# PacificBiosciences/portello

Hardware: AMD Instinct MI355X
Metric: lifted HiFi reads/sec (whole node) (higher is better)
Workload: dtype int32; 1 GPU; wgs30x; reads_total=2000000, reads_this_rank=2000000, read_len_mean=15000, items_per_gpu=2065417, in_ops_per_gpu=62827345, out_ops_per_gpu=56590310, large_items_per_gpu=0, mid_items_per_gpu=0, retry_items_per_gpu=0, lane_items_per_gpu=2065417, heavy_lane_items_per_gpu=0, seq_fmt=bam4, parallelism=one read set, 20 Mb windows dealt to 1 ranks by input ops, gather=none, launched_by=single process

## Files before the change

### portello_amd/csrc/engine.hip

```cpp
#include <hip/hip_runtime.h>

#include <plo_wave.hpp>
#include <stdio.h>
#include <string.h>

#include <algorithm>
#include <chrono>
#include <map>
#include <mutex>
#include <string>
#include <vector>

#include "enumerate.hpp"
#include "finish_core.hpp"
#include "records_core.hpp"
#include "index_pack.hpp"
#include "inflate.hpp"
#include "deflate.hpp"
#include "lift_core.hpp"
#include "lane_core.hpp"
#include "lane_stream.hpp"

using namespace plo;

// ... 96 lines not shown
        bad |= (uint32_t)__shfl_xor((int)bad, (int)d, 64);
    }
    if (!live || sub != 0) return;
    if (bad) n = 0;
    seg_reflen[s] = (int)part;
    seg_readlen[s] = rpart > 0xfffffffeull ? 0xffffffffu : (uint32_t)rpart;
    seg_nm[s] = (c1 - c0) - pairs;
    seg_cnt[s] = n;
}

__global__ void k_item_emit(DevIndex ix, DevBatch bt, DevWork wk, uint32_t stages, const uint32_t *seg_off, int *seg_reflen, uint32_t item_cap, uint32_t *err) {
    uint32_t s = blockIdx.x * blockDim.x + threadIdx.x;
    if (s >= bt.n_segs) return;
    const uint32_t o0 = seg_off[s], o1 = seg_off[s + 1];
    if (o1 > item_cap) {
        if (o1 > o0) atomicOr(err, (uint32_t)VERR_CAP);
        return;
    }
    const int ref_len = seg_reflen[s];
    SegInfo si;
    seg_info_level0(si, bt, wk, stages, s);
    if (o0 == o1) return;
    seg_info_level1(si, ix, bt, wk, stages, s);
    emit_segment_items(ix, wk, stages, s, o0, (long long)ref_len, si);
}

__global__ __launch_bounds__(64) void k_map_build(const uint32_t *seg_cigar, const uint32_t *seg_cigar_off, const int64_t *seg_pos, uint32_t n_segments,
                                                  const uint32_t *kv_off, KV *kv, int *counts) {
    for (uint32_t g = blockIdx.x; g < n_segments; g += gridDim.x) {
        const uint32_t c0 = seg_cigar_off[g], c1 = seg_cigar_off[g + 1];
        const int cnt = build_segment_map_wave(seg_cigar + c0, c1 - c0, (long long)seg_pos[g], kv ? kv + kv_off[g] : nullptr);
        if (counts && threadIdx.x == 0) counts[g] = cnt;
    }
}

__global__ void k_item_desc(DevIndex ix, DevBatch bt, DevWork wk, uint32_t stages, const uint32_t *in_seg, const uint32_t *in_cseg,
                            uint32_t *err) {
    uint32_t i = blockIdx.x * blockDim.x + threadIdx.x;
    if (i >= wk.n_items) return;
    uint32_t seg = in_seg[i];
    {
        bool ok = seg < bt.n_segs;
        if (ok) {
            uint32_t contig = bt.seg_contig[seg];
            ok = contig < ix.n_contigs && in_cseg[i] < ix.contig_seg_off[contig + 1] - ix.contig_seg_off[contig];
        }
        if (!ok) {
            atomicOr(err, (uint32_t)VERR_INDEX);
            wk.item_cls[i] = 2u;
            wk.item_nin[i] = 0u;
            return;
        }
    }
    build_item_desc(ix, bt, wk, stages, i, seg, in_cseg[i], segment_ref_len(bt, seg));
}

constexpr int SCAN_THREADS = 256;
constexpr int SCAN_PER_THREAD = 8;
constexpr int SCAN_BLOCK = SCAN_THREADS * SCAN_PER_THREAD;

__device__ __forceinline__ unsigned block_scan_incl(unsigned v, unsigned *wave_tot , unsigned &block_total) {
    int lane = threadIdx.x & 63, w = threadIdx.x >> 6;
    unsigned inc = (unsigned)wv::scan_add((int)v);
    if (lane == 63) wave_tot[w] = inc;
    __syncthreads();
    unsigned base = 0;
// ... 1160 lines not shown
        d_chrom_ref, d_chrom_ref_len, d_read_len;
    DevBuf o_status, o_flip, o_mapq, o_chrom, o_pos, o_coff, o_clen, o_cigar, o_dense_off, o_cigar_dense, wave_stats;
    DevBuf fast_blk;
    bool fast_timing = false;
    bool scan_chain = false;
    bool fast_fuse = true;
    bool phase_events = true;
    bool fast_no_events = false;
    DevBuf i_read_rev, i_read_len, i_read_off, i_seq, i_seg_read, i_seg_contig, i_seg_pos, i_seg_fwd, i_seg_coff, i_cigar,
        i_item_seg, i_item_cseg;
    HostBuf h_item_seg, h_item_cseg, h_status, h_flip, h_mapq, h_chrom, h_pos, h_coff, h_clen, h_cigar, h_counters, h_miss, h_side;
    hipEvent_t ev[7] = {nullptr, nullptr, nullptr, nullptr, nullptr, nullptr, nullptr};
    hipStream_t copy_stream = nullptr;
    hipEvent_t ev_seq = nullptr;
    hipEvent_t ev_cls = nullptr;
    bool seq_pending = false;
    bool ev_big = false, ev_mid = false;
    uint64_t dense_total = 0;
    plo_timing timing{};
    unsigned long long phase_cycles[12] = {0};
    int window = 256, big_thresh = 176, cap = 320;
    bool adaptive = true;
    int n_cus = 256;
    int tile_waves = TILE_WAVES;
    bool small_window_tight = false;
    int lane_max_w = 192;
    int lane_capw = 3072;
    bool lane_sort = true;
    DevBuf lane_ticket;
    uint32_t lane_epoch = 0;
    int lane_static_rounds = 0;
    int lane_tail_rounds = 1;
    int lane_kvs = LANE_KVS;
    bool lane_h16 = false;
    bool lane_stats = false;
    int lane_sort_window = LANE_SORT_WINDOW;
    bool lane_budget = false;
    int lane_budget_window = 512;
    bool lane_stream = true;
    bool fast = true;
    uint32_t fast_ns_cap = 0, fast_item_cap = 0, fast_n0 = 0, fast_n1 = 0;
    uint32_t fast_ref_items = 0, fast_ref_ns = 0;
    bool fast_launch_bound = true;
    uint32_t item_cap_now = 0;
    uint32_t fast_extra_syncs = 0;
    bool fast_light_only = false;
    uint32_t lane_groups_cap = 0;
    int lane_heavy_min = -1;
    int lane_heavy_ratio = 50000;
    int lane_stream_ratio = 30000;
    int mid_waves = 16;
    int mid_cap_max = 4096;
};

#define HIP_TRY(ctx, call)                                                                      \
    do {                                                                                        \
        hipError_t _e = (call);                                                                 \
        if (_e != hipSuccess) {                                                                 \
            (ctx)->err = std::string(#call) + ": " + hipGetErrorString(_e);                     \
            return (_e == hipErrorOutOfMemory) ? PLO_ERR_OUT_OF_MEMORY : PLO_ERR_HIP;           \
        }                                                                                       \
    } while (0)

static thread_local std::string g_index_err;

template <class T>
// ... 57 lines not shown
        if (upload(tmp, cg, &d_cg) != hipSuccess || upload(tmp, cgoff, &d_cgoff) != hipSuccess || upload(tmp, spos, &d_pos) != hipSuccess ||
            upload(tmp, cnt, &d_cnt) != hipSuccess) {
            drop_tmp();
            return fail(PLO_ERR_HIP);
        }
        if (ns) hipLaunchKernelGGL(k_map_build, dim3(std::min<uint32_t>(ns, 65535u * 16u)), dim3(64), 0, 0, d_cg, d_cgoff, d_pos, ns, (const uint32_t *)nullptr,
                                   (KV *)nullptr, (int *)d_cnt);
        if (hipMemcpy(cnt.data(), d_cnt, cnt.size() * 4, hipMemcpyDeviceToHost) != hipSuccess) {
            drop_tmp();
            return fail(PLO_ERR_HIP);
        }
        ix->host.cs_kv_off.assign(ns + 1, 0);
        for (uint32_t g = 0; g < ns; ++g) {
            if (cnt[g] < 0) {
                g_index_err = "contig segment coordinate outside the 31-bit BAM range or invalid CIGAR op code";
                drop_tmp();
                return fail(PLO_ERR_RANGE);
            }
            ix->host.cs_kv_off[g + 1] = ix->host.cs_kv_off[g] + (uint32_t)cnt[g];
        }
        if (upload(ix->owned, h.cs_kv_off, &d.cs_kv_off) != hipSuccess) {
            drop_tmp();
            return fail(PLO_ERR_HIP);
        }
        void *kvp = nullptr;
        if (hipMalloc(&kvp, std::max<size_t>((size_t)h.cs_kv_off[ns] * sizeof(KV), 16)) != hipSuccess) {
            drop_tmp();
            return fail(PLO_ERR_OUT_OF_MEMORY);
        }
        ix->owned.push_back(kvp);
        d.kv = (const KV *)kvp;
        if (ns) hipLaunchKernelGGL(k_map_build, dim3(std::min<uint32_t>(ns, 65535u * 16u)), dim3(64), 0, 0, d_cg, d_cgoff, d_pos, ns, d.cs_kv_off, (KV *)kvp,
                                   (int *)nullptr);
        hipError_t e = hipDeviceSynchronize();
        drop_tmp();
        if (e != hipSuccess) return fail(PLO_ERR_HIP);
    }
    if (upload(ix->owned, h.cs_chrom, &d.cs_chrom) != hipSuccess) return fail(PLO_ERR_HIP);
    if (upload(ix->owned, h.cs_is_fwd, &d.cs_is_fwd) != hipSuccess) return fail(PLO_ERR_HIP);
    if (upload(ix->owned, h.cs_mapq, &d.cs_mapq) != hipSuccess) return fail(PLO_ERR_HIP);
    if (upload(ix->owned, h.cs_start, &d.cs_start) != hipSuccess) return fail(PLO_ERR_HIP);
    if (upload(ix->owned, h.cs_end, &d.cs_end) != hipSuccess) return fail(PLO_ERR_HIP);
    if (upload(ix->owned, h.contig_seg_off, &d.contig_seg_off) != hipSuccess) return fail(PLO_ERR_HIP);
    if (upload(ix->owned, h.contig_len, &d.contig_len) != hipSuccess) return fail(PLO_ERR_HIP);
    if (upload(ix->owned, h.chrom_len, &d.chrom_len) != hipSuccess) return fail(PLO_ERR_HIP);
    d.n_contigs = desc->n_contigs;
    d.n_segments = desc->n_segments;
    d.n_chroms = desc->n_chroms;
    std::vector<const uint8_t *> chrom_ptr(desc->n_chroms, nullptr), rev_ptr(desc->n_contigs, nullptr);
    for (uint32_t c = 0; c < desc->n_chroms; ++c) {
        const uint8_t *src = desc->chrom_seq[c];
        if (!src && desc->chrom_len[c] > 0) return fail(PLO_ERR_INVALID_ARG);
        if (desc->seq_mem == PLO_MEM_DEVICE) {
            chrom_ptr[c] = src;
        } else {
            void *p = nullptr;
            size_t bytes = std::max<size_t>((size_t)desc->chrom_len[c], 16);
            if (hipMalloc(&p, bytes) != hipSuccess) return fail(PLO_ERR_OUT_OF_MEMORY);
            ix->owned.push_back(p);
            if (desc->chrom_len[c] > 0 && hipMemcpy(p, src, (size_t)desc->chrom_len[c], hipMemcpyHostToDevice) != hipSuccess)
                return fail(PLO_ERR_HIP);
            chrom_ptr[c] = (const uint8_t *)p;
        }
    }
    for (uint32_t c = 0; c < desc->n_contigs; ++c) {
        const uint8_t *src = desc->rev_contig_seq ? desc->rev_contig_seq[c] : nullptr;
// ... 73 lines not shown
    (void)hipFuncSetAttribute((const void *)k_lift_tiles, hipFuncAttributeMaxDynamicSharedMemorySize, 160 * 1024);
    (void)hipFuncSetAttribute((const void *)k_lift_tiles_sp, hipFuncAttributeMaxDynamicSharedMemorySize, 160 * 1024);
    (void)hipFuncSetAttribute((const void *)k_lift_tiles_c256, hipFuncAttributeMaxDynamicSharedMemorySize, 160 * 1024);
    (void)hipFuncSetAttribute((const void *)k_lift_retry_sp, hipFuncAttributeMaxDynamicSharedMemorySize, 160 * 1024);
    (void)hipFuncSetAttribute((const void *)k_lift_mid_sp<8>, hipFuncAttributeMaxDynamicSharedMemorySize, 160 * 1024);
    (void)hipFuncSetAttribute((const void *)k_lift_mid_sp<16>, hipFuncAttributeMaxDynamicSharedMemorySize, 160 * 1024);
    if (getenv("PLO_DEBUG")) {
        for (int cap : {256, 320, 384, 512}) {
            int nb = -1;
            size_t lds = ((tile_mem_bytes(cap) + 15) & ~(size_t)15) * TILE_WAVES;
            hipError_t e = hipOccupancyMaxActiveBlocksPerMultiprocessor(&nb, (const void *)k_lift_tiles, TILE_WAVES * 64, lds);
            fprintf(stderr, "[plo] cap %d: dynamic LDS %zu B/block -> %d blocks/CU (%s)\n", cap, lds, nb, hipGetErrorString(e));
        }
    }
    (void)hipFuncSetAttribute((const void *)k_lift_mid<8>, hipFuncAttributeMaxDynamicSharedMemorySize, 160 * 1024);
    (void)hipFuncSetAttribute((const void *)k_lift_mid<16>, hipFuncAttributeMaxDynamicSharedMemorySize, 160 * 1024);
    if (const char *e = getenv("PLO_MID_WAVES")) {
        int v = atoi(e);
        c->mid_waves = v >= 16 ? 16 : (v >= 8 ? 8 : 0);
    }
    if (const char *e = getenv("PLO_MID_CAP")) c->mid_cap_max = std::min(4096, std::max(256, atoi(e) & ~63));
    (void)hipFuncSetAttribute((const void *)k_lift_retry, hipFuncAttributeMaxDynamicSharedMemorySize, 160 * 1024);
    (void)hipFuncSetAttribute((const void *)k_lift_lanes, hipFuncAttributeMaxDynamicSharedMemorySize, 160 * 1024);
    (void)hipFuncSetAttribute((const void *)k_lift_lanes_sp, hipFuncAttributeMaxDynamicSharedMemorySize, 160 * 1024);
    (void)hipFuncSetAttribute((const void *)k_lift_lanes_stats, hipFuncAttributeMaxDynamicSharedMemorySize, 160 * 1024);
    (void)hipFuncSetAttribute((const void *)k_lift_lanes16, hipFuncAttributeMaxDynamicSharedMemorySize, 160 * 1024);
    (void)hipFuncSetAttribute((const void *)k_lift_lanes16_stats, hipFuncAttributeMaxDynamicSharedMemorySize, 160 * 1024);
    if (const char *e = getenv("PLO_LANE_MAX_W")) c->lane_max_w = atoi(e);
    if (const char *e = getenv("PLO_LANE_SORT")) c->lane_sort = atoi(e) != 0;
    if (const char *e = getenv("PLO_LANE_STATIC")) c->lane_static_rounds = atoi(e);
    if (const char *e = getenv("PLO_LANE_STATS")) c->lane_stats = atoi(e) != 0;
    if (const char *e = getenv("PLO_LANE_H16")) c->lane_h16 = atoi(e) != 0;
    if (const char *e = getenv("PLO_LANE_TAIL")) c->lane_tail_rounds = std::max(0, atoi(e));
    if (const char *e = getenv("PLO_LANE_KVS")) c->lane_kvs = std::min(LANE_KVS_MAX, std::max(64, atoi(e) & ~63));
    if (!c->lane_h16) c->lane_kvs = std::min(c->lane_kvs, LANE_KVS);
    if (const char *e = getenv("PLO_LANE_SORT_WINDOW")) c->lane_sort_window = c->lane_budget_window = std::min(2048, std::max(64, atoi(e) & ~63));
    if (const char *e = getenv("PLO_LANE_BUDGET")) c->lane_budget = atoi(e) != 0;
    if (const char *e = getenv("PLO_LANE_HEAVY_MIN")) c->lane_heavy_min = atoi(e);
    if (const char *e = getenv("PLO_LANE_HEAVY_RATIO")) c->lane_heavy_ratio = std::max(0, atoi(e));
    if (const char *e = getenv("PLO_LANE_STREAM_RATIO")) c->lane_stream_ratio = std::max(1, atoi(e));
    if (const char *e = getenv("PLO_FAST_PATH")) c->fast = atoi(e) != 0;
    if (const char *e = getenv("PLO_SCAN_CHAIN")) c->scan_chain = atoi(e) != 0;
    if (const char *e = getenv("PLO_FAST_LAUNCH_BOUND")) c->fast_launch_bound = atoi(e) != 0;
    if (const char *e = getenv("PLO_FAST_FUSE")) c->fast_fuse = atoi(e) != 0;
    if (const char *e = getenv("PLO_RECORDS_BYTECOPY")) c->rec_bytecopy = atoi(e) != 0;
    if (const char *e = getenv("PLO_PHASE_EVENTS")) c->phase_events = atoi(e) != 0;
    if (const char *e = getenv("PLO_LANE_CAPW")) c->lane_capw = std::min(40000, std::max(64, atoi(e))) & ~3;
    if (c->lane_max_w + LANE_SLACK > c->lane_capw) c->lane_max_w = c->lane_capw - LANE_SLACK;
    if (const char *e = getenv("PLO_TILE_WAVES")) c->tile_waves = std::min(TILE_WAVES, std::max(1, atoi(e)));
    if (const char *e = getenv("PLO_WINDOW")) c->window = std::max(16, atoi(e)), c->adaptive = false;
    if (const char *e = getenv("PLO_BIG_THRESH")) c->big_thresh = std::max(1, atoi(e)), c->adaptive = false;
    if (const char *e = getenv("PLO_CAP")) c->cap = std::max(64, atoi(e)), c->adaptive = false;
    *out = c;
    return PLO_OK;
}

void plo_ctx_destroy(plo_ctx *c) {
    if (!c) return;
    (void)hipSetDevice(c->ix->device);
    (void)hipStreamSynchronize(c->stream);
    DevBuf *bufs[] = {&c->f_flag, &c->f_bin, &c->f_end, &c->f_prim, &c->f_isoff, &c->f_iqoff, &c->f_iread, &c->f_nl, &c->f_pitem,
                      &c->f_uflag, &c->f_rsoff, &c->f_rqoff, &c->f_su, &c->f_qu, &c->f_soff, &c->f_qoff, &c->f_rseq, &c->f_rqual, &c->f_fflag, &c->f_frank, &c->f_flist, &c->sa_len, &c->sa_off, &c->sa_text, &c->r_plan, &c->r_size, &c->r_start, &c->r_partial, &c->r_recoff, &c->r_out, &c->r_err, &c->z_slots, &c->z_size, &c->z_off, &c->z_partial, &c->z_tok, &c->z_out, &c->z_err,
                      &c->item_region, &c->lane_groups, &c->lane_ticket, &c->misc, &c->whist, &c->cls_partial, &c->lane_scratch, &c->item_cls, &c->retry_list, &c->perm, &c->nin_p, &c->seg_reflen, &c->seg_readlen, &c->seg_nm, &c->seg_cnt, &c->seg_off, &c->scan_partial, &c->item_seg, &c->item_cseg, &c->item_nin, &c->op_prefix,
                      &c->counters, &c->big_list, &c->huge_list, &c->verr, &c->scratch, &c->tile_lo, &c->d_n_m, &c->d_in_off, &c->d_n_in, &c->d_pos1,
                      &c->d_w0, &c->d_w1, &c->d_kv0, &c->d_kv1, &c->d_flags, &c->d_contig, &c->d_seq_len, &c->d_seq_off, &c->d_shift_ref,
                      &c->d_shift_ref_len, &c->d_chrom_ref, &c->d_chrom_ref_len, &c->d_read_len, &c->o_status, &c->o_flip, &c->o_mapq, &c->o_chrom, &c->o_pos,
// ... 400 lines not shown
            for (; b > 0; --b) {
                if (above + hist[b] > allow) break;
                above += hist[b];
            }
            int thresh = std::min(std::max(176, (b + 1) * WHIST_STEP), (WHIST_BINS - 1) * WHIST_STEP);
            c->big_thresh = thresh;
            c->cap = thresh <= 176 && !sp && !getenv("PLO_NO_SMALL_CAP") ? TILE_CAP_SMALL : (thresh <= 256 ? 320 : (thresh + 144 + 63) & ~63);
            c->window = c->cap - (c->cap == TILE_CAP_SMALL && !c->small_window_tight ? 32 : 64);
            c->tile_waves = c->cap <= 320 ? TILE_WAVES : (c->cap <= 448 ? 2 : 1);
            if (getenv("PLO_DEBUG_GEOMETRY"))
                fprintf(stderr, "[plo] batch geometry: thresh %d cap %d window %d tile_waves %d (max weight %u, %llu items beyond the 0.2 %% cut)\n", thresh, c->cap,
                        c->window, c->tile_waves, max_nin, above);
        }
    }
    const uint32_t n_tiles = total_ops / (uint32_t)c->window + 1;
    if (n_items > n_small && !heavy_lanes) {
        HIP_TRY(c, c->tile_lo.ensure((size_t)(n_tiles + 1) * 4));
        hipLaunchKernelGGL(k_tile_bounds, dim3((n_tiles + 1 + 255) / 256), dim3(256), 0, st, (const uint32_t *)c->op_prefix.as<uint32_t>(),
                           n_items, n_tiles, c->window, n_small, c->tile_lo.as<uint32_t>());
    }
    wk.tile_lo = c->tile_lo.as<uint32_t>();
    wk.n_small = n_small;
    HIP_TRY(c, hipEventRecord(c->ev[1], st));

    uint32_t lane_gs = 64, lane_nblk = 0;
    const size_t lane_lds = (size_t)(c->lane_capw + 2 * c->lane_kvs) * 4 * LANE_WAVES;
    if (n_small) {
        int occ = 1;
        if (hipOccupancyMaxActiveBlocksPerMultiprocessor(&occ, sp ? (const void *)k_lift_lanes_sp : (const void *)k_lift_lanes, LANE_WAVES * 64, lane_lds) != hipSuccess || occ < 1)
            occ = 1;
        const uint32_t n0 = h_cls[0], n1 = h_cls[1];
        const uint32_t slots = (uint32_t)(c->n_cus * occ) * LANE_WAVES;
        while (lane_gs > 8u && (n0 + lane_gs / 2 - 1) / (lane_gs / 2) + (n1 + lane_gs / 2 - 1) / (lane_gs / 2) <= slots) lane_gs >>= 1;
        if (const char *e = getenv("PLO_LANE_GROUP")) lane_gs = std::min(64u, std::max(1u, (uint32_t)atoi(e)));
        const uint32_t groups = (n0 + lane_gs - 1) / lane_gs + (n1 + lane_gs - 1) / lane_gs;
        lane_nblk = std::min<uint32_t>((groups + LANE_WAVES - 1) / LANE_WAVES, (uint32_t)(c->n_cus * occ));
        lane_nblk = (lane_nblk + 7u) & ~7u;
    }
    size_t want_cigar = (size_t)all_ops * 2 + (size_t)n_items * 8 + 4096 + (size_t)std::min<uint32_t>(n_tiles + 1024, (uint32_t)c->n_cus * 16) * SLAB_OPS +
                        (size_t)lane_nblk * LANE_WAVES * SLAB_OPS;
    if (c->o_cigar.cap < want_cigar * 4) HIP_TRY(c, c->o_cigar.ensure(want_cigar * 4));

    if (c->seq_pending) {
        HIP_TRY(c, hipStreamWaitEvent(st, c->ev_seq, 0));
        c->seq_pending = false;
    }
    unsigned long long *hc = c->h_counters.as<unsigned long long>();
    uint32_t n_big = 0, n_retry = 0, n_mid = 0, n_huge = 0, n_miss = 0, heavy_kernel = 0;
    float miss_ms = 0.f;
    for (int attempt = 0;; ++attempt) {
        wk.out_cigar = c->o_cigar.as<uint32_t>();
        wk.out_cap = c->o_cigar.cap / 4;
        HIP_TRY(c, hipMemsetAsync(c->counters.p, 0, CNT_N * 8, st));
        if (attempt == 0) HIP_TRY(c, hipEventRecord(c->ev[1], st));
        wk.slab_pre = 0;
        wk.slab_offset = 0;
        if (n_small) {
            const uint32_t n0 = h_cls[0], n1 = h_cls[1];
            const bool budget = c->lane_sort && wk.item_region && lane_gs == 64u;
            uint32_t lane_groups_cap_now = 0;
            if (attempt == 0 && c->lane_sort) {
                const uint32_t ch = (uint32_t)(budget ? c->lane_budget_window : c->lane_sort_window);
                const uint32_t chunks = (n0 + ch - 1) / ch + (n1 + ch - 1) / ch;
                uint32_t *n_groups_dev = c->misc.as<uint32_t>() + 32;
                if (budget) {
                    const uint32_t per_group = std::min<uint32_t>(64u, std::max<uint32_t>(1u, (uint32_t)c->lane_capw / (uint32_t)std::max(1, c->lane_max_w)));
                    const size_t max_groups = (size_t)chunks * (ch / per_group + 2);
// ... 322 lines not shown
    HIP_TRY(c, c->h_counters.ensure(FB_BYTES));
    uint8_t *const fb = c->fast_blk.as<uint8_t>();
    uint32_t *const misc_d = (uint32_t *)fb, *const verr_d = (uint32_t *)(fb + FB_VERR);
    unsigned long long *const counters_d = (unsigned long long *)(fb + FB_COUNTERS);
    const bool ev_on = c->phase_events;
    if (ev_on) HIP_TRY(c, hipEventRecord(c->ev[0], st));
    HIP_TRY(c, hipMemsetAsync(fb, 0, fb_bytes, st));
    hipLaunchKernelGGL(k_seg_count, dim3((unsigned)(((unsigned long long)ns * SEG_LANES + 255) / 256)), dim3(256), 0, st, ix, bt, c->seg_cnt.as<uint32_t>(),
                       c->seg_reflen.as<int>(), c->seg_readlen.as<uint32_t>(), c->seg_nm.as<uint32_t>(), verr_d);
    if (chain) {
        hipLaunchKernelGGL(k_scan_chain, dim3(scan_nb), dim3(SCAN_THREADS), 0, st, (const uint32_t *)c->seg_cnt.as<uint32_t>(), ns, c->seg_off.as<uint32_t>(),
                           (unsigned long long *)(fb + FB_BYTES), (uint32_t *)(fb + FB_TICKET));
    } else {
        plo_status s = scan_u32(c, c->seg_cnt.as<uint32_t>(), ns, c->seg_off.as<uint32_t>());
        if (s != PLO_OK) return s;
    }
    const uint32_t *n_dev = c->seg_off.as<uint32_t>() + ns, *totals_dev = misc_d;
    DevWork wk;
    fill_work(c, wk, cap);
    wk.counters = counters_d;
    hipLaunchKernelGGL(k_item_emit, dim3((ns + 255) / 256), dim3(256), 0, st, ix, bt, wk, stages, (const uint32_t *)c->seg_off.as<uint32_t>(), c->seg_reflen.as<int>(),
                       cap, verr_d);
    const uint32_t cls_nb = (cap + CLS_BLOCK - 1) / CLS_BLOCK;
    HIP_TRY(c, c->cls_partial.ensure((size_t)std::max(1u, cls_nb) * 6 * 4));
    hipLaunchKernelGGL(k_cls_hist, dim3(cls_nb), dim3(CLS_THREADS), 0, st, (const uint32_t *)c->item_cls.as<uint32_t>(), (const uint32_t *)c->item_nin.as<uint32_t>(), cap,
                       cls_nb, c->cls_partial.as<uint32_t>(), n_dev);
    hipLaunchKernelGGL(k_permute2_s, dim3(cls_nb), dim3(CLS_THREADS), 0, st, (const uint32_t *)c->item_cls.as<uint32_t>(), (const uint32_t *)c->item_nin.as<uint32_t>(),
                       (const uint32_t *)c->cls_partial.as<uint32_t>(), misc_d, cap, cls_nb, c->perm.as<uint32_t>(), c->nin_p.as<uint32_t>(),
                       c->adaptive ? (uint32_t)((WHIST_BINS - 1) * WHIST_STEP) : 0xffffffffu, n_dev);
    if (ev_on) HIP_TRY(c, hipEventRecord(c->ev[1], st));
    uint32_t lane_gs = 64, lane_nblk = 0;
    const size_t lane_lds = (size_t)(c->lane_capw + 2 * c->lane_kvs) * 4 * LANE_WAVES;
    {
        int occ = 1;
        if (hipOccupancyMaxActiveBlocksPerMultiprocessor(&occ, (const void *)k_lift_lanes, LANE_WAVES * 64, lane_lds) != hipSuccess || occ < 1) occ = 1;
        const uint32_t n0 = c->fast_n0, n1 = c->fast_n1, slots = (uint32_t)(c->n_cus * occ) * LANE_WAVES;
        while (lane_gs > 8u && (n0 + lane_gs / 2 - 1) / (lane_gs / 2) + (n1 + lane_gs / 2 - 1) / (lane_gs / 2) <= slots) lane_gs >>= 1;
        if (const char *e = getenv("PLO_LANE_GROUP")) lane_gs = std::min(64u, std::max(1u, (uint32_t)atoi(e)));
        const uint32_t groups = cap / lane_gs + 2;
        lane_nblk = std::min<uint32_t>((groups + LANE_WAVES - 1) / LANE_WAVES, (uint32_t)(c->n_cus * occ));
        lane_nblk = (lane_nblk + 7u) & ~7u;
    }
    const uint32_t ch = (uint32_t)c->lane_sort_window;
    hipLaunchKernelGGL(k_chunk_sort_w, dim3((cap / ch + 2u + 3u) / 4u), dim3(256), 0, st, c->perm.as<uint32_t>(), (const uint32_t *)c->d_n_m.as<uint32_t>(),
                       (const uint32_t *)c->d_w0.as<uint32_t>(), (const uint32_t *)c->d_w1.as<uint32_t>(), 0u, 0u, ch, totals_dev);
    wk.out_cigar = c->o_cigar.as<uint32_t>();
    wk.out_cap = c->o_cigar.cap / 4;
    wk.slab_pre = 1u;
    wk.slab_offset = (unsigned long long)lane_nblk * LANE_WAVES * SLAB_OPS;
    wk.n_small = cap;
    wk.lane_n_groups = misc_d + 32;
    wk.stat_base = 0;
    uint32_t stat_used = lane_nblk * LANE_WAVES;
    if (wk.slab_offset + SLAB_OPS > wk.out_cap) {
        fallback = true;
        return PLO_OK;
    }
    if (c->seq_pending) {
        HIP_TRY(c, hipStreamWaitEvent(st, c->ev_seq, 0));
        c->seq_pending = false;
    }
    lane_ticket_arm(c, wk, (c->fast_n0 + lane_gs - 1) / lane_gs + (c->fast_n1 + lane_gs - 1) / lane_gs, lane_nblk * LANE_WAVES);
    hipLaunchKernelGGL(lane_kernel_of(c, stages, false), dim3(lane_nblk), dim3(LANE_WAVES * 64), lane_lds, st, ix, bt, wk, stages, 0u, 0u, lane_gs, c->lane_capw, totals_dev);
    HIP_TRY(c, hipGetLastError());
    if (ev_on) HIP_TRY(c, hipEventRecord(c->ev[4], st));
    {
        const int retry_cap = 320;
        const uint32_t lds = (uint32_t)((tile_mem_bytes(retry_cap) + 15) & ~(size_t)15), nw = (uint32_t)c->n_cus * 2u;
#ifdef PLO_PHASE_TIMING
        const bool fuse = false;
#else
// ... 847 lines not shown
```

### portello_amd/csrc/enumerate.hpp

```cpp
#pragma once
#include <plo_wave.hpp>

#include "lift_types.hpp"

namespace plo {

#ifdef PLO_EMULATOR
alignas(16) static const uint32_t plo_safe_words[8] = {0, 0, 0, 0, 0, 0, 0, 0};
#else
alignas(16) static __device__ const uint32_t plo_safe_words[8] = {0, 0, 0, 0, 0, 0, 0, 0};
#endif

#ifdef PLO_EMULATOR
#define PLO_LEVEL_END(...)
#else
#define PLO_LV_(x) "v"(x)
#define PLO_LV1(a) PLO_LV_(a)
#define PLO_LV2(a, ...) PLO_LV_(a), PLO_LV1(__VA_ARGS__)
#define PLO_LV3(a, ...) PLO_LV_(a), PLO_LV2(__VA_ARGS__)
#define PLO_LV4(a, ...) PLO_LV_(a), PLO_LV3(__VA_ARGS__)
#define PLO_LV5(a, ...) PLO_LV_(a), PLO_LV4(__VA_ARGS__)
#define PLO_LV6(a, ...) PLO_LV_(a), PLO_LV5(__VA_ARGS__)
#define PLO_LV7(a, ...) PLO_LV_(a), PLO_LV6(__VA_ARGS__)
#define PLO_LV8(a, ...) PLO_LV_(a), PLO_LV7(__VA_ARGS__)
#define PLO_LV9(a, ...) PLO_LV_(a), PLO_LV8(__VA_ARGS__)
#define PLO_LV_N(_1, _2, _3, _4, _5, _6, _7, _8, _9, n, ...) PLO_LV##n
#define PLO_LEVEL_END(...) asm volatile("" ::PLO_LV_N(__VA_ARGS__, 9, 8, 7, 6, 5, 4, 3, 2, 1)(__VA_ARGS__))
#endif

PLO_DEV long long segment_ref_len(const DevBatch &bt, uint32_t seg) {
    uint32_t c0 = bt.seg_cigar_off[seg], c1 = bt.seg_cigar_off[seg + 1];
    long long r = 0;
    for (uint32_t i = c0; i < c1; ++i) {
        uint32_t c = bt.cigar[i];
        if ((0x18D >> (c & 15u)) & 1) r += (long long)(c >> 4);
    }
    return r;
}

PLO_DEV uint32_t segment_read_len_sat(const DevBatch &bt, uint32_t seg) {
    uint32_t c0 = bt.seg_cigar_off[seg], c1 = bt.seg_cigar_off[seg + 1];
    unsigned long long r = 0;
    for (uint32_t i = c0; i < c1; ++i) {
        uint32_t c = bt.cigar[i];
        if ((0x1B3 >> (c & 15u)) & 1) r += (unsigned long long)(c >> 4);
    }
    return r > 0xfffffffeull ? 0xffffffffu : (uint32_t)r;
}

PLO_DEV uint32_t segment_n_merged(const DevBatch &bt, uint32_t seg) {
    uint32_t c0 = bt.seg_cigar_off[seg], c1 = bt.seg_cigar_off[seg + 1];
    uint32_t n = 0;
    bool prev = false;
    for (uint32_t i = c0; i < c1; ++i) {
        const bool m = ((0x181u >> (bt.cigar[i] & 15u)) & 1u) != 0u;
        n += (m && prev) ? 0u : 1u;
        prev = m;
    }
    return n;
}
// ... 40 lines not shown
        int mid = (int)(((unsigned)lo + (unsigned)hi) >> 1);
        if (kv[mid].key < x)
            lo = mid + 1;
        else
            hi = mid;
    }
    return lo;
}

PLO_DEV int kv_lower_bound_near(const KV *kv, int lo, int hi, int x) {
    {
        int k[8];
#pragma unroll
        for (int j = 0; j < 8; ++j) k[j] = (lo + j < hi ? kv + (lo + j) : (const KV *)plo_safe_words)->key;
        int c = 0;
#pragma unroll
        for (int j = 0; j < 8; ++j) c += ((lo + j < hi) & (k[j] < x)) ? 1 : 0;
        if (c < 8 || lo + 8 >= hi) return lo + c;
        lo += 8;
    }
    int step = 1;
    while (lo < hi) {
        int probe = lo + step - 1;
        if (probe >= hi) break;
        if (kv[probe].key < x) {
            lo = probe + 1;
            step <<= 1;
        } else {
            hi = probe;
            break;
        }
    }
    return kv_lower_bound(kv, lo, hi, x);
}

PLO_HD int build_segment_map(const uint32_t *cigar, uint32_t n, long long ref_pos, KV *out) {
    long long read_pos = 0, match_len = 0;
    int cnt = 0;
    int last_key = -1;
    bool bad = false;
    for (uint32_t i = 0; i <= n; ++i) {
        uint32_t c = i < n ? cigar[i] : 4u;
        int t = (int)(c & 15u);
        long long len = (long long)(c >> 4);
        if (t > 8) bad = true;
        bool is_m = (t == OP_M || t == OP_EQ || t == OP_X);
        if (is_m) {
            match_len += len;
        } else if (match_len > 0) {
            if (read_pos > 0x7ffffff0LL || ref_pos > 0x7ffffff0LL || ref_pos - match_len < 0) {
                bad = true;
            } else {
                int k0 = (int)(read_pos - match_len), v0 = (int)(ref_pos - match_len), k1 = (int)read_pos;
                if (cnt > 0 && last_key == k0) {
                    if (out) out[cnt - 1].val = v0;
                } else {
                    if (out) {
                        out[cnt].key = k0;
                        out[cnt].val = v0;
                    }
                    ++cnt;
                }
                if (out) {
                    out[cnt].key = k1;
                    out[cnt].val = NONE32;
                }
// ... 90 lines not shown
    uint64_t seq_off, revseq;
    bool seg_fwd, read_rev;
};
PLO_DEV void seg_info_level0(SegInfo &s, const DevBatch &bt, const DevWork &wk, uint32_t stages, uint32_t seg) {
    s.contig = bt.seg_contig[seg];
    s.read = bt.seg_read[seg];
    s.in_off = bt.seg_cigar_off[seg];
    s.n_in = bt.seg_cigar_off[seg + 1];
    s.pos = (long long)bt.seg_pos[seg];
    s.n_m = wk.seg_nm ? wk.seg_nm[seg] : 0u;
    s.read_len = wk.seg_readlen ? wk.seg_readlen[seg] : 0u;
    const uint32_t sf = (stages & PLO_STAGE_STRAND) ? (uint32_t)bt.seg_is_fwd[seg] : 0u;
    PLO_LEVEL_END(s.contig, s.read, s.in_off, s.n_in, s.pos, s.n_m, s.read_len, sf);
    s.seg_fwd = sf != 0u;
    s.n_in -= s.in_off;
}
PLO_DEV void seg_info_level1(SegInfo &s, const DevIndex &ix, const DevBatch &bt, const DevWork &wk, uint32_t stages, uint32_t seg) {
    s.g0 = ix.contig_seg_off[s.contig];
    s.g1 = ix.contig_seg_off[s.contig + 1];
    s.contig_len = ix.contig_len[s.contig];
    s.revseq = ix.contig_revseq ? (uint64_t)(uintptr_t)ix.contig_revseq[s.contig] : 0ull;
    s.seq_len = bt.read_seq_len[s.read];
    s.seq_off = bt.read_seq_off[s.read];
    const uint32_t rr = (stages & PLO_STAGE_STRAND) ? (uint32_t)bt.read_is_reverse[s.read] : 0u;
    PLO_LEVEL_END(s.g0, s.g1, s.contig_len, s.revseq, s.seq_len, s.seq_off, rr);
    s.read_rev = rr != 0u;
    if (!wk.seg_nm) s.n_m = segment_n_merged(bt, seg);
    if (!wk.seg_readlen) s.read_len = segment_read_len_sat(bt, seg);
}
struct CsegInfo {
    int start, end;
    uint32_t kv0, kv1, chrom;
    uint8_t is_fwd, mapq;
};
PLO_DEV CsegInfo cseg_info(const DevIndex &ix, uint32_t gseg) {
    CsegInfo c;
    c.start = ix.cs_start[gseg];
    c.end = ix.cs_end[gseg];
    c.kv0 = ix.cs_kv_off[gseg];
    c.kv1 = ix.cs_kv_off[gseg + 1];
    c.chrom = ix.cs_chrom[gseg];
    const uint32_t f = ix.cs_is_fwd[gseg], q = ix.cs_mapq[gseg];
    PLO_LEVEL_END(c.start, c.end, c.kv0, c.kv1, c.chrom, f, q);
    c.is_fwd = (uint8_t)f;
    c.mapq = (uint8_t)q;
    return c;
}

PLO_DEV void build_item_desc(const DevIndex &ix, const DevWork &wk, uint32_t stages, uint32_t i, uint32_t seg, uint32_t cseg, long long ref_len,
                             const SegInfo &s, const CsegInfo &c) {
    const bool contig_fwd = c.is_fwd != 0;
    bool flip = false, rev = false;
    if (stages & PLO_STAGE_STRAND) {
        const bool changes = s.read_rev == s.seg_fwd;
        flip = (!contig_fwd) != changes;
        rev = !contig_fwd;
    }
    const long long pos1 = rev ? (long long)s.contig_len - (s.pos + ref_len) : s.pos;
    const int kv0 = (int)c.kv0, kv1 = (int)c.kv1;
    const long long lo = pos1 < -0x7fffffffLL ? -0x7fffffffLL : pos1;
    const long long hi = pos1 + ref_len > 0x7fffffffLL ? 0x7fffffffLL : pos1 + ref_len;
    int slo = kv0, shi = kv1;
    kv_upper_bound_narrow(ix.kv, slo, shi, (int)lo);
    const uint64_t chrom_ref = (uint64_t)(uintptr_t)ix.chrom_seq[c.chrom];
    const int chrom_ref_len = ix.chrom_len[c.chrom];
    const int ub = kv_upper_bound_tail(ix.kv, slo, shi, (int)lo);
    PLO_LEVEL_END(chrom_ref, chrom_ref_len, ub);
    const int w0 = ub - 1 > kv0 ? ub - 1 : kv0;
    const int w1 = kv_lower_bound_near(ix.kv, w0, kv1, (int)hi);
    const bool do_shift = (stages & PLO_STAGE_LSHIFT) && (!(stages & PLO_STAGE_STRAND) || !contig_fwd);
    const bool merges = do_shift || (stages & PLO_STAGE_LIFTOVER);
    const int region = lane_region_dwords((int)(merges ? s.n_m : s.n_in), w0, w1);
    wk.item_seg[i] = seg;
    wk.item_cseg[i] = cseg;
    wk.item_nin[i] = (uint32_t)item_weight((int)s.n_in, w0, w1, kv1);
    wk.item_cls[i] = (do_shift ? 1u : 0u) | ((wk.lane_max_w < 0 || region > wk.lane_max_w) ? 2u : 0u);
    if (wk.item_region) wk.item_region[i] = (uint32_t)region;
    wk.d.n_m[i] = s.n_m;
    wk.d.in_off[i] = s.in_off;
    wk.d.n_in[i] = s.n_in;
    wk.d.pos1[i] = (int)pos1;
    wk.d.w0[i] = (uint32_t)w0;
    wk.d.w1[i] = (uint32_t)w1;
    wk.d.kv0[i] = (uint32_t)kv0;
    wk.d.kv1[i] = (uint32_t)kv1;
    wk.d.flags[i] = (rev ? (uint32_t)ITF_REV : 0u) | (flip ? (uint32_t)ITF_FLIP : 0u) | (contig_fwd ? (uint32_t)ITF_CONTIG_FWD : 0u);
    wk.d.contig[i] = s.contig;
    wk.d.seq_len[i] = s.seq_len;
    wk.d.seq_off[i] = s.seq_off;
    wk.d.shift_ref[i] = s.revseq;
    wk.d.shift_ref_len[i] = s.contig_len;
    wk.d.chrom_ref[i] = chrom_ref;
    wk.d.chrom_ref_len[i] = chrom_ref_len;
    wk.d.read_len[i] = s.read_len;
    wk.flip[i] = (uint8_t)flip;
// ... 89 lines not shown
```

### portello_amd/csrc/lift_types.hpp

```cpp
#pragma once
#include <stdint.h>

#include "../../include/portello_liftover.h"

namespace plo {

enum : int { OP_M = 0, OP_I = 1, OP_D = 2, OP_N = 3, OP_S = 4, OP_H = 5, OP_P = 6, OP_EQ = 7, OP_X = 8 };
constexpr int NONE32 = (int)0x80000000;
constexpr int IMAX = 0x7fffffff;
constexpr int ITEM_NEED_BIG = 0xFF;
constexpr int MAXI = 64;
constexpr uint32_t sparse_header_bytes(uint32_t seq_len) { return ((((seq_len + 1023u) >> 10) * 8u) + 15u) & ~15u; }

struct alignas(8) KV {
    int key;
    int val;
};

struct DevIndex {
    const KV *kv;
    const uint32_t *cs_kv_off;
    const uint32_t *cs_chrom;
    const uint8_t *cs_is_fwd;
    const uint8_t *cs_mapq;
    const int *cs_start;
    const int *cs_end;
    const uint32_t *contig_seg_off;
    const int *contig_len;
    const uint8_t *const *contig_revseq;
    const uint8_t *const *chrom_seq;
    const int *chrom_len;
    uint32_t n_contigs, n_segments, n_chroms;
};

struct DevBatch {
    const uint8_t *read_is_reverse;
    const uint32_t *read_seq_len;
    const uint64_t *read_seq_off;
    const uint8_t *seq;
    int seq_fmt;
    uint64_t seq_bytes;
    const uint32_t *seg_read;
    const uint32_t *seg_contig;
    const int64_t *seg_pos;
    const uint8_t *seg_is_fwd;
    const uint32_t *seg_cigar_off;
    const uint32_t *cigar;
    uint32_t n_reads, n_segs;
};

enum { CNT_CIGAR = 0, CNT_OVERFLOW = 1, CNT_NBIG = 2, CNT_ALGO_BYTES = 3, CNT_IN_OPS = 4, CNT_ERROR = 5, CNT_OUT_OPS = 6, CNT_NRETRY = 7, CNT_PHASE0 = 8, CNT_NHUGE = 20, CNT_NMISS = 21, CNT_LANE_ACT = 22, CNT_LANE_TRIPS = 23, CNT_N = 24 };

struct ItemDesc {
    uint32_t *in_off;
    uint32_t *n_in;
    uint32_t *n_m;
    int *pos1;
    uint32_t *w0, *w1;
    uint32_t *kv0, *kv1;
    uint32_t *flags;
    uint32_t *contig;
    uint32_t *seq_len;
    uint64_t *seq_off;
    uint64_t *shift_ref;
    int *shift_ref_len;
// ... 51 lines not shown
```

Measured before the change: 1.499 billion reads/s.

## Add per-segment bucket table to narrow KV binary search in item descriptor

Builds, at index load time, a per-contig-segment bucket table that maps a shifted reference position to a KV lower-bound index. Item descriptor setup uses it to bracket the KV range before the narrowing binary search, so each lookup needs fewer dependent global loads. It also caches the lane-kernel occupancy query and the PLO_LANE_GROUP env parse so they are not repeated on every call. The cost is extra index memory and build time, plus a header load per item.

```diff
diff --git a/portello_amd/csrc/engine.hip b/portello_amd/csrc/engine.hip
--- a/portello_amd/csrc/engine.hip
+++ b/portello_amd/csrc/engine.hip
@@ -152,6 +152,10 @@
         const int cnt = build_segment_map_wave(seg_cigar + c0, c1 - c0, (long long)seg_pos[g], kv ? kv + kv_off[g] : nullptr);
         if (counts && threadIdx.x == 0) counts[g] = cnt;
     }
+}
+
+__global__ __launch_bounds__(64) void k_btab_build(const KV *kv, const uint32_t *kv_off, const uint32_t *tab_off, uint32_t n_segments, BTabHdr *hdr, uint32_t *tab) {
+    for (uint32_t g = blockIdx.x; g < n_segments; g += gridDim.x) btab_build_segment(kv, kv_off[g], kv_off[g + 1], tab_off[g], hdr + g, tab, threadIdx.x, 64u);
 }
 
 __global__ void k_item_desc(DevIndex ix, DevBatch bt, DevWork wk, uint32_t stages, const uint32_t *in_seg, const uint32_t *in_cseg,
@@ -1378,6 +1382,9 @@
     int lane_static_rounds = 0;
     int lane_tail_rounds = 1;
     int lane_kvs = LANE_KVS;
+    uint32_t lane_group_env = 0;
+    size_t fast_occ_lds = ~(size_t)0;
+    int fast_occ = 1;
     bool lane_h16 = false;
     bool lane_stats = false;
     int lane_sort_window = LANE_SORT_WINDOW;
@@ -1501,6 +1508,31 @@
         d.kv = (const KV *)kvp;
         if (ns) hipLaunchKernelGGL(k_map_build, dim3(std::min<uint32_t>(ns, 65535u * 16u)), dim3(64), 0, 0, d_cg, d_cgoff, d_pos, ns, d.cs_kv_off, (KV *)kvp,
                                    (int *)nullptr);
+        const char *bt_env = getenv("PLO_BTAB");
+        if (ns && !(bt_env && atoi(bt_env) == 0)) {
+            std::vector<uint32_t> toff(ns + 1, 0);
+            unsigned long long tot = 0;
+            for (uint32_t g = 0; g < ns; ++g) {
+                toff[g] = (uint32_t)tot;
+                tot += btab_entries(h.cs_kv_off[g + 1] - h.cs_kv_off[g]);
+            }
+            toff[ns] = (uint32_t)tot;
+            const uint32_t *d_toff = nullptr;
+            void *hdr = nullptr, *tab = nullptr;
+            if (upload(tmp, toff, &d_toff) != hipSuccess || hipMalloc(&hdr, (size_t)ns * sizeof(BTabHdr)) != hipSuccess) {
+                drop_tmp();
+                return fail(PLO_ERR_OUT_OF_MEMORY);
+            }
+            ix->owned.push_back(hdr);
+            if (hipMalloc(&tab, std::max<size_t>((size_t)tot * 4, 16)) != hipSuccess) {
+                drop_tmp();
+                return fail(PLO_ERR_OUT_OF_MEMORY);
+            }
+            ix->owned.push_back(tab);
+            hipLaunchKernelGGL(k_btab_build, dim3(std::min<uint32_t>(ns, 65535u * 16u)), dim3(64), 0, 0, d.kv, d.cs_kv_off, d_toff, ns, (BTabHdr *)hdr, (uint32_t *)tab);
+            d.cs_btab = (const BTabHdr *)hdr;
+            d.btab = (const uint32_t *)tab;
+        }
         hipError_t e = hipDeviceSynchronize();
         drop_tmp();
         if (e != hipSuccess) return fail(PLO_ERR_HIP);
@@ -1640,6 +1672,7 @@
     if (const char *e = getenv("PLO_LANE_STATS")) c->lane_stats = atoi(e) != 0;
     if (const char *e = getenv("PLO_LANE_H16")) c->lane_h16 = atoi(e) != 0;
     if (const char *e = getenv("PLO_LANE_TAIL")) c->lane_tail_rounds = std::max(0, atoi(e));
+    if (const char *e = getenv("PLO_LANE_GROUP")) c->lane_group_env = std::min(64u, std::max(1u, (uint32_t)atoi(e)));
     if (const char *e = getenv("PLO_LANE_KVS")) c->lane_kvs = std::min(LANE_KVS_MAX, std::max(64, atoi(e) & ~63));
     if (!c->lane_h16) c->lane_kvs = std::min(c->lane_kvs, LANE_KVS);
     if (const char *e = getenv("PLO_LANE_SORT_WINDOW")) c->lane_sort_window = c->lane_budget_window = std::min(2048, std::max(64, atoi(e) & ~63));
@@ -2106,7 +2139,7 @@
         const uint32_t n0 = h_cls[0], n1 = h_cls[1];
         const uint32_t slots = (uint32_t)(c->n_cus * occ) * LANE_WAVES;
         while (lane_gs > 8u && (n0 + lane_gs / 2 - 1) / (lane_gs / 2) + (n1 + lane_gs / 2 - 1) / (lane_gs / 2) <= slots) lane_gs >>= 1;
-        if (const char *e = getenv("PLO_LANE_GROUP")) lane_gs = std::min(64u, std::max(1u, (uint32_t)atoi(e)));
+        if (c->lane_group_env) lane_gs = c->lane_group_env;
         const uint32_t groups = (n0 + lane_gs - 1) / lane_gs + (n1 + lane_gs - 1) / lane_gs;
         lane_nblk = std::min<uint32_t>((groups + LANE_WAVES - 1) / LANE_WAVES, (uint32_t)(c->n_cus * occ));
         lane_nblk = (lane_nblk + 7u) & ~7u;
@@ -2495,11 +2528,16 @@
     uint32_t lane_gs = 64, lane_nblk = 0;
     const size_t lane_lds = (size_t)(c->lane_capw + 2 * c->lane_kvs) * 4 * LANE_WAVES;
     {
-        int occ = 1;
-        if (hipOccupancyMaxActiveBlocksPerMultiprocessor(&occ, (const void *)k_lift_lanes, LANE_WAVES * 64, lane_lds) != hipSuccess || occ < 1) occ = 1;
+        if (c->fast_occ_lds != lane_lds) {
+            int q = 1;
+            if (hipOccupancyMaxActiveBlocksPerMultiprocessor(&q, (const void *)k_lift_lanes, LANE_WAVES * 64, lane_lds) != hipSuccess || q < 1) q = 1;
+            c->fast_occ = q;
+            c->fast_occ_lds = lane_lds;
+        }
+        const int occ = c->fast_occ;
         const uint32_t n0 = c->fast_n0, n1 = c->fast_n1, slots = (uint32_t)(c->n_cus * occ) * LANE_WAVES;
         while (lane_gs > 8u && (n0 + lane_gs / 2 - 1) / (lane_gs / 2) + (n1 + lane_gs / 2 - 1) / (lane_gs / 2) <= slots) lane_gs >>= 1;
-        if (const char *e = getenv("PLO_LANE_GROUP")) lane_gs = std::min(64u, std::max(1u, (uint32_t)atoi(e)));
+        if (c->lane_group_env) lane_gs = c->lane_group_env;
         const uint32_t groups = cap / lane_gs + 2;
         lane_nblk = std::min<uint32_t>((groups + LANE_WAVES - 1) / LANE_WAVES, (uint32_t)(c->n_cus * occ));
         lane_nblk = (lane_nblk + 7u) & ~7u;
diff --git a/portello_amd/csrc/enumerate.hpp b/portello_amd/csrc/enumerate.hpp
--- a/portello_amd/csrc/enumerate.hpp
+++ b/portello_amd/csrc/enumerate.hpp
@@ -24,8 +24,11 @@
 #define PLO_LV7(a, ...) PLO_LV_(a), PLO_LV6(__VA_ARGS__)
 #define PLO_LV8(a, ...) PLO_LV_(a), PLO_LV7(__VA_ARGS__)
 #define PLO_LV9(a, ...) PLO_LV_(a), PLO_LV8(__VA_ARGS__)
-#define PLO_LV_N(_1, _2, _3, _4, _5, _6, _7, _8, _9, n, ...) PLO_LV##n
-#define PLO_LEVEL_END(...) asm volatile("" ::PLO_LV_N(__VA_ARGS__, 9, 8, 7, 6, 5, 4, 3, 2, 1)(__VA_ARGS__))
+#define PLO_LV10(a, ...) PLO_LV_(a), PLO_LV9(__VA_ARGS__)
+#define PLO_LV11(a, ...) PLO_LV_(a), PLO_LV10(__VA_ARGS__)
+#define PLO_LV12(a, ...) PLO_LV_(a), PLO_LV11(__VA_ARGS__)
+#define PLO_LV_N(_1, _2, _3, _4, _5, _6, _7, _8, _9, _10, _11, _12, n, ...) PLO_LV##n
+#define PLO_LEVEL_END(...) asm volatile("" ::PLO_LV_N(__VA_ARGS__, 12, 11, 10, 9, 8, 7, 6, 5, 4, 3, 2, 1)(__VA_ARGS__))
 #endif
 
 PLO_DEV long long segment_ref_len(const DevBatch &bt, uint32_t seg) {
@@ -132,6 +135,42 @@
         }
     }
     return kv_lower_bound(kv, lo, hi, x);
+}
+
+PLO_HD uint32_t btab_room(uint32_t n) { return (n + 1u) / 2u; }
+PLO_HD uint32_t btab_entries(uint32_t n) { return n ? btab_room(n) + 1u : 0u; }
+PLO_HD BTabHdr btab_header(uint32_t n, int first, int last, uint32_t off) {
+    const unsigned long long span1 = (unsigned long long)((long long)last - (long long)first);
+    const uint32_t room = btab_room(n);
+    uint32_t sh = 0;
+    while ((span1 >> sh) + 1ull > (unsigned long long)room) ++sh;
+    BTabHdr h;
+    h.base = first;
+    h.shift = sh;
+    h.off = off;
+    h.nb = (uint32_t)(span1 >> sh) + 1u;
+    return h;
+}
+PLO_HD uint32_t btab_bucket(const BTabHdr &h, int x) {
+    const long long d = (long long)x - (long long)h.base;
+    const unsigned long long b = d > 0 ? (unsigned long long)d >> h.shift : 0ull;
+    return b < (unsigned long long)h.nb ? (uint32_t)b : h.nb - 1u;
+}
+PLO_DEV void btab_bracket(const uint32_t *tab, const BTabHdr &h, int x, int &lo, int &hi) {
+    const bool have = tab != nullptr && h.nb != 0u;
+    const uint32_t *const bp = have ? tab + h.off + btab_bucket(h, x) : (const uint32_t *)plo_safe_words;
+    const uint32_t b0 = bp[0], b1 = bp[1];
+    PLO_LEVEL_END(b0, b1);
+    if (have) lo = (int)b0, hi = (int)b1;
+}
+PLO_DEV void btab_build_segment(const KV *kv, uint32_t kv0, uint32_t kv1, uint32_t off, BTabHdr *hdr, uint32_t *tab, uint32_t l, uint32_t nl) {
+    BTabHdr h;
+    h.base = 0, h.shift = 0u, h.off = off, h.nb = 0u;
+    if (kv1 > kv0) h = btab_header(kv1 - kv0, kv[kv0].key, kv[kv1 - 1u].key, off);
+    if (l == 0u) *hdr = h;
+    if (!h.nb) return;
+    for (uint32_t b = l; b <= h.nb; b += nl)
+        tab[off + b] = b == h.nb ? kv1 : (uint32_t)kv_lower_bound(kv, (int)kv0, (int)kv1, (int)((long long)h.base + ((long long)b << h.shift)));
 }
 
 PLO_HD int build_segment_map(const uint32_t *cigar, uint32_t n, long long ref_pos, KV *out) {
@@ -288,6 +327,7 @@
     int start, end;
     uint32_t kv0, kv1, chrom;
     uint8_t is_fwd, mapq;
+    BTabHdr bt;
 };
 PLO_DEV CsegInfo cseg_info(const DevIndex &ix, uint32_t gseg) {
     CsegInfo c;
@@ -297,7 +337,8 @@
     c.kv1 = ix.cs_kv_off[gseg + 1];
     c.chrom = ix.cs_chrom[gseg];
     const uint32_t f = ix.cs_is_fwd[gseg], q = ix.cs_mapq[gseg];
-    PLO_LEVEL_END(c.start, c.end, c.kv0, c.kv1, c.chrom, f, q);
+    c.bt = *(ix.cs_btab ? ix.cs_btab + gseg : (const BTabHdr *)plo_safe_words);
+    PLO_LEVEL_END(c.start, c.end, c.kv0, c.kv1, c.chrom, f, q, c.bt.base, c.bt.shift, c.bt.off, c.bt.nb);
     c.is_fwd = (uint8_t)f;
     c.mapq = (uint8_t)q;
     return c;
@@ -317,6 +358,7 @@
     const long long lo = pos1 < -0x7fffffffLL ? -0x7fffffffLL : pos1;
     const long long hi = pos1 + ref_len > 0x7fffffffLL ? 0x7fffffffLL : pos1 + ref_len;
     int slo = kv0, shi = kv1;
+    btab_bracket(ix.btab, c.bt, (int)lo, slo, shi);
     kv_upper_bound_narrow(ix.kv, slo, shi, (int)lo);
     const uint64_t chrom_ref = (uint64_t)(uintptr_t)ix.chrom_seq[c.chrom];
     const int chrom_ref_len = ix.chrom_len[c.chrom];
diff --git a/portello_amd/csrc/lift_types.hpp b/portello_amd/csrc/lift_types.hpp
--- a/portello_amd/csrc/lift_types.hpp
+++ b/portello_amd/csrc/lift_types.hpp
@@ -17,6 +17,11 @@
     int val;
 };
 
+struct alignas(16) BTabHdr {
+    int base;
+    uint32_t shift, off, nb;
+};
+
 struct DevIndex {
     const KV *kv;
     const uint32_t *cs_kv_off;
@@ -31,6 +36,8 @@
     const uint8_t *const *chrom_seq;
     const int *chrom_len;
     uint32_t n_contigs, n_segments, n_chroms;
+    const BTabHdr *cs_btab = nullptr;
+    const uint32_t *btab = nullptr;
 };
 
 struct DevBatch {
```

New measurement: 1.497 billion reads/s. No clear change (-0.2%).
